# FrancisGregoryNg/Gaussian_Process_Optimization

Hardware: AMD Instinct MI355X
Metric: GP fit+predict iters/sec at N=16384 D=8 (higher is better)
Workload: dtype f64; 1 GPU; C3 (BASELINE.json configs[2]): N=16384, D=8 RBF iso, fit (K, Cholesky, alpha, LML) + predict mean/var at M=10000 candidates + EI arg-best; candidates_total=10000, candidates_this_rank=10000, entry_point=gp_fit_predict, kernel=RBF, fit=replicated on every rank (does not shard, SURVEY.md 8e), torch_imported=False, launcher=single process, emulate_fp64=0

## Files before the change

gaussian_process_optimization_amd/csrc/api_core.hip:

```cpp
#include "api_internal.h"

thread_local std::string g_err;

static thread_local bool g_note_set = false;
static thread_local std::string g_note_msg;

int fail(int code, const char *fmt, ...) {
    char buf[512];
    va_list ap;
    va_start(ap, fmt);
    vsnprintf(buf, sizeof buf, fmt, ap);
    va_end(ap);
    g_err = buf;
    if (g_note_set) {
        g_err += " [after: " + g_note_msg + "]";
        g_note_set = false;
    }
    return code;
}

void gp_note_hip(hipError_t e, const char *what, const char *file, int line) {
    if (e == hipSuccess || g_note_set) return;
    char buf[512];
    snprintf(buf, sizeof buf, "%s -> %s (%s:%d)", what, hipGetErrorString(e), file, line);
// ... 333 lines not shown
        g->panel_tiles = (int)value;
    } else if (!strcmp(name, "inner_tiles")) {
        if (value != 1 && value != 2) return fail(GP_ERR_ARG, "inner_tiles must be 1 or 2");
        g->inner_tiles = (int)value;
    } else if (!strcmp(name, "inner_min_rows")) {
        if (value < 0) return fail(GP_ERR_ARG, "inner_min_rows < 0");
        g->inner_min_rows = (int)std::min<int64_t>(value, 1 << 20);
    } else if (!strcmp(name, "own_keep_per_row")) {
        if (value < 0) return fail(GP_ERR_ARG, "own_keep_per_row < 0");
        g->own_keep_per_row = (int)std::min<int64_t>(value, 1 << 20);
    } else if (!strcmp(name, "own_keep_pipe_pct")) {
        if (value < 0 || value > 400) return fail(GP_ERR_ARG, "own_keep_pipe_pct out of range");
        g->own_keep_pipe_pct = (int)value;
    } else if (!strcmp(name, "own_keep_base")) {
        if (value < 0) return fail(GP_ERR_ARG, "own_keep_base < 0");
        g->own_keep_base = (int)std::min<int64_t>(value, 1 << 20);
    } else if (!strcmp(name, "lookahead")) {
        g->lookahead = value ? 1 : 0;
    } else if (!strcmp(name, "lookahead_min_tiles")) {
        if (value < 0) return fail(GP_ERR_ARG, "lookahead_min_tiles < 0");
        g->lookahead_min_tiles = (int)std::min<int64_t>(value, 1 << 20);
    } else if (!strcmp(name, "pipe_start_pct")) {
        if (value < -1 || value > 100) return fail(GP_ERR_ARG, "pipe_start_pct out of range");
        g->pipe_start_pct = (int)value;
    } else if (!strcmp(name, "small_below")) {
        g->small_below = (int)value;
    } else if (!strcmp(name, "profile_min_tiles")) {
        if (value < 0) return fail(GP_ERR_ARG, "profile_min_tiles < 0");
        g->profile_min_tiles = value;
    } else if (!strcmp(name, "pipe_stages_grad")) {
        if (value < 0) return fail(GP_ERR_ARG, "pipe_stages_grad < 0");
        g->pipe_stages_grad = (int)std::min<int64_t>(value, 1 << 20);
    } else if (!strcmp(name, "pipe_start_pct_grad")) {
        if (value < 0 || value > 100) return fail(GP_ERR_ARG, "pipe_start_pct_grad out of range");
        g->pipe_start_pct_grad = (int)value;
    } else if (!strcmp(name, "pipe_stages")) {
        if (value < 0) return fail(GP_ERR_ARG, "pipe_stages < 0");
        g->pipe_stages = (int)std::min<int64_t>(value, 1 << 20);
    } else if (!strcmp(name, "lauum_panels")) {
        g->lauum_panels = (int)value;
        g->wi_valid = false;
        g->li_valid = false;
        g->rows_calls_since_fit = 0;
        g->w_in_t2 = false;
    } else if (!strcmp(name, "side_alpha")) {
        g->side_alpha = (int)value;
    } else if (!strcmp(name, "pair_panels")) {
        g->pair_panels = value ? 1 : 0;
    } else if (!strcmp(name, "pair_tri")) {
        g->pair_tri = (int)value;
    } else if (!strcmp(name, "fmin_direct")) {
        g->fmin_direct = (int)value;
        g->fmin_valid = false;
    } else if (!strcmp(name, "chain_small_below")) {
        g->chain_small_below = (int)value;
    } else if (!strcmp(name, "waves8")) {
        g->waves8 = value ? 1 : 0;
    } else if (!strcmp(name, "stagger")) {
        g->stagger = (int)value;
    } else if (!strcmp(name, "supertile")) {
        if (value < 0 || value > 64) return fail(GP_ERR_ARG, "supertile out of range");
        if (g->supertile != (int)value) {
            HIPCHK(hipSetDevice(g->device));
            HIPCHK(hipDeviceSynchronize());
            for (auto &kv : g->tile_lists) hipFree(kv.second);
            g->tile_lists.clear();
        }
        g->supertile = (int)value;
    } else if (!strcmp(name, "reserve_cus")) {
        if (value != g->bulk_reserved)
            return fail(GP_ERR_ARG, "reserve_cus is fixed when the device's streams are created (%d); set GPHIP_RESERVE_CUS "
                                    "before the first gp_create", g->bulk_reserved);
    } else if (!strcmp(name, "trsm_rows64")) {
        g->trsm_rows64 = (int)value;
    } else if (!strcmp(name, "rns_interleave")) {
        rns_set_interleave((int)value);
    } else if (!strcmp(name, "rns_group_fit")) {
        if (value < 1 || value > 16) return fail(GP_ERR_ARG, "rns_group_fit must be in [1, 16]");
        g->rns_group_fit = (int)value;
    } else if (!strcmp(name, "rns_group")) {
        if (value < 1 || value > 16) return fail(GP_ERR_ARG, "rns_group must be in [1, 16]");
        g->rns_group = (int)value;
    } else if (!strcmp(name, "emulate_fit")) {
        g->emulate_fit = value ? 1 : 0;
    } else if (!strcmp(name, "emulate_fp64")) {
        g->emulate_fp64 = value ? 1 : 0;
        g->predicted = false;
    } else if (!strcmp(name, "debug_potrf_lds")) {
        if (value < 0 || value > (1 << 20)) return fail(GP_ERR_ARG, "debug_potrf_lds out of range");
        potrf_set_debug_lds((int)value);
    } else if (!strcmp(name, "debug_rows_skew")) {
        g->rows_counter_base += (unsigned int)value;
    } else if (!strcmp(name, "rows_build")) {
        if (value < -1 || value > 1) return fail(GP_ERR_ARG, "rows_build out of range (-1: by rule, 0: never, 1: at the first call)");
        g->rows_build = (int)value;
    } else if (!strcmp(name, "rows_nt")) {
        if (value < -1 || value > 1) return fail(GP_ERR_ARG, "rows_nt out of range (-1: automatic, 0, 1)");
        g->rows_nt = (int)value;
    } else if (!strcmp(name, "small_m")) {
        if (value < 0 || value > 8) return fail(GP_ERR_ARG, "small_m out of range (0..8)");
        g->small_m = value;
        g->predicted = false;
    } else if (!strcmp(name, "mc_max")) {
        if (value < GP_TILE) return fail(GP_ERR_ARG, "mc_max < 128");
        g->mc_max = round_up(value, GP_TILE);
    } else
// ... 227 lines not shown
```

gaussian_process_optimization_amd/csrc/api_factor.hip:

```cpp
#include "api_internal.h"

void build_ky(gp_ctx *g, const Members &m, bool jittered) {
    launch_kbuild(g->s, m.A, m.lda, g->dX, g->N, g->Npad, m.kp[0], m.diag[0], 0, m.nb, m.sA, m.kpt, m.diag_tab);
    if (jittered) launch_add_diag(g->s, m.A, m.lda, g->N, m.jit[0], m.nb, m.sA, m.jit_tab);
    launch_set_rhs(g->s, m.A, m.lda, g->dY, g->N, g->Npad, g->P, m.nb, m.sA);
}

static int chain_step(gp_ctx *g, hipStream_t s, const Members &m, int j, int J1, int R1) {
    double *A = m.A, *invL = m.invL;
    const long lda = m.lda;
    if (g->inner_tiles >= 2 && m.nb == 1 && j + 1 < J1 && R1 - (j + 2) >= g->inner_min_rows) {
        launch_potrf_pair(s, A, lda, j, invL, m.info);
        launch_trsm2(s, A, lda, j, invL, j + 2, R1);
        if (j + 2 < J1)
            gemm(g, s, 1, A, lda, A + (long)j * GP_TILE, lda, A + (long)j * GP_TILE, lda, 1, 2 * GP_TILE,
                 TileSet{0, R1, j + 2, J1, 1});
        return j + 2;
    }
    launch_potrf_tile(s, A, lda, j, invL, m.info, m.nb, m.sA, m.sI, 4);
    gemm(g, s, 0, A, lda, A + (long)j * GP_TILE, lda, invL + (long)j * GP_TILE * GP_TILE, GP_TILE, 0, GP_TILE,
         TileSet{j + 1, R1, j, j + 1, 0}, member_opt(m, inplace_opt(), m.sA, m.sA, m.sI));
    if (j + 1 < J1)
        gemm(g, s, 1, A, lda, A + (long)j * GP_TILE, lda, A + (long)j * GP_TILE, lda, 1, GP_TILE, TileSet{0, R1, j + 1, J1, 1},
             member_opt(m, GemmOpt(), m.sA, m.sA, m.sA));
    return j + 1;
}

void factor_buf(gp_ctx *g, const Members &m, int nt, int R1, bool side_inv) {
    const int W = g->panel_tiles;
    hipStream_t s = g->s;
    double *A = m.A;
    const long lda = m.lda;
    if (side_inv) {
        hipEvent_t e0 = la_event(g, EV_MISC, 0);
        GP_NOTE(hipEventRecord(e0, s));
        GP_NOTE(hipStreamWaitEvent(g->s_inv, e0, 0));
    }
    for (int J0 = 0; J0 < nt; J0 += W) {
        const int J1 = std::min(J0 + W, nt);
        for (int j = J0; j < J1;) j = chain_step(g, s, m, j, J1, R1);
        if (side_inv) {
            hipEvent_t eF = la_event(g, EV_CHAIN, J0 / W);
            GP_NOTE(hipEventRecord(eF, s));
            GP_NOTE(hipStreamWaitEvent(g->s_inv, eF, 0));
            build_panel_inv_one(g, g->s_inv, J0 / W, W, nt);
        }
        if (J1 < nt)
            gemm(g, s, 1, A, lda, A + (long)J0 * GP_TILE, lda, A + (long)J0 * GP_TILE, lda, 1, (J1 - J0) * GP_TILE,
                 TileSet{0, R1, J1, nt, 1}, member_opt(m, GemmOpt(), m.sA, m.sA, m.sA));
    }
    if (side_inv) {
        hipEvent_t ei = la_event(g, EV_MISC, 4);
        GP_NOTE(hipEventRecord(ei, g->s_inv));
        GP_NOTE(hipStreamWaitEvent(s, ei, 0));
    }
}

int factor(gp_ctx *g) {
    const int nt = (int)(g->Npad / GP_TILE);
    const int W = g->panel_tiles;
    const bool side = nt > W && g->s_inv;
    if (side) {
        const long PB = (long)W * GP_TILE;
        const int nJ = (nt + W - 1) / W;
        int rc;
        if ((rc = dev_realloc(&g->dInvP, &g->capInvP, (long)nJ * PB * PB))) return rc;
        if ((rc = dev_realloc(&g->dInvPw, &g->capInvPw, (long)nJ * PB * PB))) return rc;
    }
    factor_buf(g, ctx_members(g), nt, nt + 1, side);
    if (side) {
        g->invp_W = W;
        g->invp_valid = true;
        return la_events_ok(g);
    }
    return 0;
}

int factor_lookahead(gp_ctx *g, const PredPipe &pp) {
    int rc;
    if ((rc = ensure_bulk_stream(g))) return rc;
    const long lda = g->Npad;
    const int nt = (int)(g->Npad / GP_TILE);
    const int R1 = nt + 1;
    const int W = g->panel_tiles;
    double *A = g->dA;
    hipStream_t sp = g->s_panel, sb = g->s_bulk;
    hipEvent_t e0 = la_event(g, EV_MISC, 0);
    GP_NOTE(hipEventRecord(e0, g->s));
    GP_NOTE(hipStreamWaitEvent(sp, e0, 0));
    GP_NOTE(hipStreamWaitEvent(sb, e0, 0));
    const long PB = (long)W * GP_TILE;
    const int nJu = (nt + W - 1) / W;
    if ((rc = dev_realloc(&g->dInvP, &g->capInvP, (long)nJu * PB * PB))) return rc;
    if ((rc = dev_realloc(&g->dInvPw, &g->capInvPw, (long)nJu * PB * PB))) return rc;
    GP_NOTE(hipStreamWaitEvent(g->s_inv, e0, 0));
    if (pp.on) {
        GP_NOTE(hipStreamWaitEvent(g->s_pred, e0, 0));
        if (pp.init) pp.init(g->s_pred);
    }
    int next_pred = 0;
    int own_prev = nt;
    const int pstages = pp.on ? std::max(1, std::min(nJu, pp.stages)) : 0;
    const int pred_start = std::max(0, std::min(nJu - 1, nJu * pp.start_pct / 100));
    std::vector<int> pb;
    for (int j = 0; j < nt; j += W) pb.push_back(j);
    pb.push_back(nt);
    pb.push_back(nt);
    const int nJ = (int)pb.size() - 2;
    const bool emu = emu_fit_applies(g);
    RnsGeom rg;
    int *rflag = g->dInfo + 2;
    if (emu) {
        if ((rc = rns_prepare(g, g->jitter_try, &rg))) return rc;
        const long need = (long)GP_RNS_T * rg.nt256 * rg.nt256 * 65536;
        if ((rc = byte_realloc(&g->dRm, &g->capRm, need))) return rc;
    }
    const int Gf = (emu && !pp.on) ? std::max(1, std::min(g->rns_group_fit, (int)(GP_RNS_KMAX / PB))) : 1;
    hipStream_t sfar = g->s_pred;
    std::vector<char> far_issued(nJ / std::max(1, Gf) + 2, 0);
    int mid_Jg = -1, mid_end = 0, mid_first = 0, mid_base = 0, mid_next = 0;
    if (Gf > 1) GP_NOTE(hipStreamWaitEvent(sfar, e0, 0));
    const Members cm = ctx_members(g);
    for (int J = 0; J < nJ; ++J) {
        const int J0 = pb[J], J1 = pb[J + 1], J2 = pb[J + 2];
        bool bulk_recorded = false;
        for (int j = J0; j < J1;) j = chain_step(g, sp, cm, j, J1, R1);
        hipEvent_t eF = la_event(g, EV_CHAIN, J);
        GP_NOTE(hipEventRecord(eF, sp));
        const int K = (J1 - J0) * GP_TILE;
        GP_NOTE(hipStreamWaitEvent(g->s_inv, eF, 0));
        build_panel_inv_one(g, g->s_inv, J, W, nt);
        if (pp.on) {
            if (J < pstages) GP_NOTE(hipEventRecord(la_event(g, EV_INVP, J), g->s_inv));
            if (J >= pred_start) {
                for (; next_pred <= J && next_pred < pstages; ++next_pred) {
                    const int Q = next_pred, Q0 = Q * W, Q1 = std::min(Q0 + W, nt);
                    const int KQ = (Q1 - Q0) * GP_TILE;
                    const int prow = pp.trapezoid ? std::min(pp.mt, Q1) : pp.mt;
                    GP_NOTE(hipStreamWaitEvent(g->s_pred, la_event(g, EV_CHAIN, J), 0));
                    GP_NOTE(hipStreamWaitEvent(g->s_pred, la_event(g, EV_INVP, Q), 0));
                    GemmOpt o;
                    o.k_end_tri = 1;
                    o.b_sub = Q0;
                    gemm(g, g->s_pred, 0, pp.S, g->Npad, pp.T + (long)Q0 * GP_TILE, g->Npad, g->dInvP + (long)Q * PB * PB,
                         PB, 1, KQ, TileSet{0, prow, Q0, Q1, 0}, o);
                    if (Q1 < nt)
                        gemm(g, g->s_pred, 1, pp.T, g->Npad, pp.S + (long)Q0 * GP_TILE, g->Npad, A + (long)Q0 * GP_TILE, lda,
                             1, KQ, TileSet{0, prow, Q1, nt, 0});
                }
            }
        }
        if (J1 >= nt) break;
        int oc = nt;
        if (!emu && g->own_keep_per_row > 0 && J2 < nt) {
            const long n = nt - J2;
            long keep = g->own_keep_base + (long)g->own_keep_per_row * n * W / 6;
            if (pp.on && J >= pred_start && own_prev < nt) keep = keep * g->own_keep_pipe_pct / 100;
            long t_own = n * (n + 1) / 2 + n - keep;
            int c = 0;
            while (c < own_prev && (long)(c + 1) * (c + 2) / 2 + (c + 1) <= t_own) ++c;
            own_prev = c;
            oc = nt - c;
        }
        if (oc < nt && J >= 1)
            gemm(g, sp, 1, A, lda, A + (long)J0 * GP_TILE, lda, A + (long)J0 * GP_TILE, lda, 1, K, TileSet{0, R1, oc, nt, 1});
        if (J >= 1) GP_NOTE(hipStreamWaitEvent(sp, la_event(g, EV_BULK, J - 1), 0));
        gemm(g, sp, 1, A, lda, A + (long)J0 * GP_TILE, lda, A + (long)J0 * GP_TILE, lda, 1, K,
             TileSet{0, R1, J1, J2, 1});
        if (oc < nt && J == 0)
            gemm(g, sp, 1, A, lda, A + (long)J0 * GP_TILE, lda, A + (long)J0 * GP_TILE, lda, 1, K, TileSet{0, R1, oc, nt, 1});
        if (J2 < nt) {
            GP_NOTE(hipStreamWaitEvent(sb, eF, 0));
            if (emu) {
                rns_convert_panel(g, sb, rg, J, rflag);
                gemm(g, sb, 1, A, lda, A + (long)J0 * GP_TILE, lda, A + (long)J0 * GP_TILE, lda, 1, K,
                     TileSet{nt, R1, J2, nt, 0});
                auto rlaunch = [&](hipStream_t st, int Jfirst, int t0, int t1, int first, int Tend = -1) {
                    t1 = std::min(t1, nt);
                    if (t0 >= t1) return;
                    const int T0 = pb[Jfirst];
                    rns_gemm(g, st, g->dLr + (long)T0 * GP_TILE, rg.Lpitch, rg.Lplane, g->dLr + (long)T0 * GP_TILE, rg.Lpitch,
                                       rg.Lplane, g->dRm, rg.nt256, rg.nt256, rg.nt256, t0 / 2, (t1 + 1) / 2,
                                       ((Tend < 0 ? J1 : Tend) - T0) * GP_TILE, first, 1);
                };
                auto pbi = [&](int k) { return pb[std::min(k, nJ + 1)]; };
                auto rebuild_next = [&]() {
                    if (pbi(J + 2) < nt)
                        launch_rns_reconstruct256(sb, g->dRm, rg.nt256, rg.nt256, rg.nt256, pbi(J + 2), std::min(pbi(J + 3), nt),
                                                  g->Npad, A, lda, rg.back, 1);
                };
                if (Gf == 1) {
                    rlaunch(sb, J, J2, nt, J == 0 ? 1 : 0);
                    rebuild_next();
                } else {
                    const int gi = J / Gf, Jg = gi * Gf;
                    const int first = gi == 0 ? 1 : 0;
                    GP_NOTE(hipEventRecord(la_event(g, EV_CONV, J), sb));
                    rlaunch(sb, Jg, pbi(J + 2), pbi(J + 3), first);
                    rebuild_next();
                    GP_NOTE(hipEventRecord(la_event(g, EV_BULK, J), sb));
                    bulk_recorded = true;
                    if (J % Gf == Gf - 1) {
                        if (gi >= 1 && far_issued[gi - 1]) GP_NOTE(hipStreamWaitEvent(sb, la_event(g, EV_FAR, gi - 1), 0));
                        mid_Jg = Jg;
                        mid_end = J1;
                        mid_first = first;
                        mid_base = J + 3;
                        mid_next = 0;
                        if (pbi(J + 3 + Gf) < nt) {
                            GP_NOTE(hipStreamWaitEvent(sfar, la_event(g, EV_CONV, J), 0));
                            rlaunch(sfar, Jg, pbi(J + 3 + Gf), nt, first);
                            GP_NOTE(hipEventRecord(la_event(g, EV_FAR, gi), sfar));
                            far_issued[gi] = true;
                        }
                    }
                    if (mid_Jg >= 0 && mid_next < Gf) {
                        rlaunch(sb, mid_Jg, pbi(mid_base + mid_next), pbi(mid_base + mid_next + 1), mid_first, mid_end);
                        ++mid_next;
                    }
                }
            } else {
// ... 95 lines not shown

int fit_impl(gp_ctx *g, int maxtries, int pipe, int include_noise) {
    HIPCHK(hipSetDevice(g->device));
    QuiesceOnError guard{g};
    const long N = g->N, Npad = g->Npad;
    const int P = g->P;
    const int nt_ = (int)(Npad / GP_TILE);
    const long mcpad = pipe == 1 ? round_up(g->M, GP_TILE) : (pipe == 2 ? Npad : 0);
    PredPipe pp;
    if (pipe) {
        int rc;
        const int W = std::min(g->panel_tiles, nt_);
        const long PB = (long)W * GP_TILE;
        const int nJ = (nt_ + W - 1) / W;
        if (pipe == 1 && (rc = ensure_out(g))) return rc;
        if ((rc = dev_realloc(&g->dT, &g->capT, mcpad * Npad))) return rc;
        if ((rc = dev_realloc(&g->dT2, &g->capT2, mcpad * Npad))) return rc;
        if (pipe == 2 && (rc = dev_realloc(&g->dWi, &g->capWi, Npad * Npad))) return rc;
        if ((rc = dev_realloc(&g->dInvP, &g->capInvP, (long)nJ * PB * PB))) return rc;
        if ((rc = dev_realloc(&g->dInvPw, &g->capInvPw, (long)nJ * PB * PB))) return rc;
        pp.on = true;
        pp.mt = (int)(mcpad / GP_TILE);
        pp.T = g->dT;
        pp.S = g->dT2;
        pp.trapezoid = (pipe == 2);
        pp.stages = pipe == 2 ? (g->pipe_stages_grad > 0 ? g->pipe_stages_grad : std::max(1, (nJ * 36 + 50) / 100))
                              : (g->pipe_stages > 0 ? g->pipe_stages : std::max(1, (nJ * 14 + 50) / 100) + (nJ <= 12 ? 1 : 0));
        pp.start_pct = pipe == 2 ? g->pipe_start_pct_grad : (g->pipe_start_pct >= 0 ? g->pipe_start_pct : (nJ <= 24 ? 32 : 40));
    }
    double diag_add, diag0;
    ky_diag(g->kp, g->noise, &diag_add, &diag0);
    g->nphases = 0;
    g->emu_off_call = false;
    g->fitted = false;
    g->fmin_valid = false;
    g->wi_valid = false;
    g->li_valid = false;
    g->rows_calls_since_fit = 0;
    g->w_in_t2 = false;
    g->invp_valid = false;
    g->lr_valid = false;
    g->predicted = false;

    double jitter = 0.0;
    int tries = 0;
    int info = 0;
    for (;;) {
        g->lr_valid = false;
        g->jitter_try = jitter;
        int ph = phase_begin(g, "kbuild", 0.0, 8.0 * N * g->D + 8.0 * (double)N * N / 2);
        Members m = ctx_members(g);
        m.diag = &diag_add;
        m.jit = &jitter;
        build_ky(g, m, jitter != 0.0);
        phase_end(g, ph);
        HIPCHK(hipMemsetAsync(g->dInfo, 0, sizeof(int) * 4, g->s));
        if (pipe == 1) {
            pp.init = [g, mcpad, N, Npad](hipStream_t st) {
                launch_cross_k(st, g->dT, Npad, g->dXs, g->M, mcpad, g->dX, N, Npad, g->kp);
            };
            ph = phase_begin(g, "cholesky+cand_solve", (double)N * N * N / 3.0 + (double)N * N * g->M, 0.0);
            int rcf = factor_lookahead(g, pp);
            if (rcf) return rcf;
        } else if (pipe == 2) {
            ph = phase_begin(g, "cholesky+potri_stages", (double)N * N * N / 3.0, 0.0);
            pp.init = [g, Npad](hipStream_t st) { launch_set_identity(st, g->dT, Npad, Npad); };
            int rcf = factor_lookahead(g, pp);
            if (rcf) return rcf;
        } else {
            ph = phase_begin(g, "cholesky", (double)N * N * N / 3.0, 0.0);
            if (g->lookahead && nt_ > g->panel_tiles && (nt_ > g->lookahead_min_tiles || emu_fit_applies(g))) {
                int rcf = factor_lookahead(g);
                if (rcf) return rcf;
            } else {
                int rcf = factor(g);
                if (rcf) return rcf;
            }
        }
        phase_end(g, ph);
        HIPCHK(hipMemcpyAsync(&info, g->dInfo, sizeof(int), hipMemcpyDeviceToHost, g->s));
        GP_SYNC(g->s);
        if (g->emulate_fp64 && !g->emu_off_call && info == 0) {
            int bad = 0;
            HIPCHK(hipMemcpy(&bad, g->dInfo + 2, sizeof(int), hipMemcpyDeviceToHost));
            if (bad) {
                g->emu_off_call = true;
                ++g->emu_fallbacks;
                g->nphases = 0;
                g->invp_valid = false;
                continue;
            }
        }
        if (info == 0) break;
        g->invp_valid = false;
        const int rcl = ladder_step(diag0, maxtries, info, &jitter, &tries);
        if (rcl == GP_ERR_NOT_PD_DIAG) return fail(rcl, "not pd: non-positive diagonal elements");
        if (rcl) {
            g_err = "not positive definite, even with jitter.";
            return rcl;
        }
        g->nphases = 0;
    }
    g->jitter = jitter;
    bool side_alpha = false;
    if (pipe) {
        const int W = std::min(g->panel_tiles, nt_);
        const int nJ = (nt_ + W - 1) / W;
        if (g->pipe_done < nJ) {
            int phr = phase_begin(g, pipe == 2 ? "potri_solve_rest" : "cand_solve_rest", 0.0, 0.0);
            int rci = ensure_panel_inv(g);
            if (rci) return rci;
            hipEvent_t eI = la_event(g, EV_MISC, 5);
            if (g->s_inv && g->side_alpha) GP_NOTE(hipEventRecord(eI, g->s));
            solve_rows(g, ctx_members(g), (int)(mcpad / GP_TILE), pipe == 2 ? 1 : 0, g->pipe_done);
            if (g->s_inv && g->side_alpha) {
                GP_NOTE(hipStreamWaitEvent(g->s_inv, eI, 0));
                alpha_lml(g, g->s_inv, ctx_members(g));
                GP_NOTE(hipEventRecord(la_event(g, EV_MISC, 6), g->s_inv));
                side_alpha = true;
            }
            phase_end(g, phr);
        }
        if (pipe == 2) {
            int rcl = wi_lauum(g);
            if (rcl) return rcl;
// ... 73 lines not shown
```

gaussian_process_optimization_amd/csrc/api_internal.h:

```cpp
#pragma once
#include "gphip_internal.h"
#include "../../include/gphip.h"

#include <hip/hip_ext.h>
#include <rccl/rccl.h>

#include <algorithm>
#include <array>
#include <cmath>
#include <cstdarg>
#include <cstdio>
#include <cstdlib>
#include <cstring>
#include <functional>
#include <map>
#include <mutex>
#include <set>
#include <string>
#include <vector>

extern thread_local std::string g_err;
int fail(int code, const char *fmt, ...);

#define HIPCHK(x)                                                                                   \
// ... 81 lines not shown
    bool li_valid = false;
    double *dRows = nullptr;
    long capRows = 0;
    unsigned int *dRowsCounter = nullptr;
    double *hRowsOut = nullptr;
    double rows_ticket = 0.0;
    unsigned int rows_counter_base = 0;
    std::vector<double> lp_cache;
    int lp_cache_nb = -1;
    long rows_fused_calls = 0, rows_fallback_calls = 0;
    long rows_calls_since_fit = 0;
    int rows_build = -1;
    int rows_nt = -1;
    double *dLp = nullptr;
    double *dX2 = nullptr, *dK2 = nullptr;
    long capX2 = 0, capK2 = 0;
    long capLp = 0;
    double *dCov = nullptr;
    long capCov = 0;
    double *dInvP = nullptr, *dInvPw = nullptr;
    long capInvP = 0, capInvPw = 0;
    int invp_W = 0;
    bool invp_valid = false;
    double *dDm = nullptr, *dDv = nullptr, *dDacq = nullptr;
    long capD = 0;
    int panel_tiles = 6;
    int lookahead = 1;
    int inner_min_rows = 0;
    int own_keep_per_row = 36, own_keep_base = 200;
    int own_keep_pipe_pct = 0;
    int inner_tiles = 1;
    int lookahead_min_tiles = 40;
    int reserve_cus = 32;
    long mc_max = 16384;
    long small_m = 8;
    Phase phases[MAX_PHASES];
    int nphases = 0;
    bool profiling = false;
    int profile_class = 0;
    std::vector<hipEvent_t> gemm_events;
    std::vector<hipEvent_t> rns_events;
    size_t rns_ev_used = 0;
    double rns_ops = 0.0;
    std::vector<long> gemm_tiles;
    std::map<std::array<int, 5>, short *> tile_lists;
    int supertile = 8;
    int small_below = 1400;
    int chain_small_below = 400;
    int lauum_panels = 1;
    int side_alpha = 1;
    int pair_panels = 1;
    int pair_tri = 2;
    int fmin_direct = 0;
    int trsm_rows64 = 32;
    int waves8 = 1;
    int stagger = 3;
    int pipe_stages_grad = 0, pipe_start_pct_grad = 40;
    int pipe_stages = 0;
    int pipe_done = 0;
    int pipe_start_pct = -1;
    std::vector<int> gemm_K;
    size_t gemm_ev_used = 0;
    long gemm_launches = 0;
    double gemm_flops = 0.0;
    double gemm_flops_all = 0.0;
    long profile_min_tiles = 1024;
    ncclComm_t comm = nullptr;
    int rank = 0, nranks = 1;
    double *dComm = nullptr;
    long capComm = 0;
    int emulate_fp64 = 0;
    int rns_group = 8;
    int rns_group_fit = 8;
    signed char *dLr = nullptr, *dSr = nullptr, *dRr = nullptr;
    signed char *dRm = nullptr;
    signed char *dWr = nullptr;
    long capWr = 0;
    long capLr = 0, capSr = 0, capRr = 0, capRm = 0;
    bool lr_valid = false;
    std::vector<char> lr_done;
    int lr_W = 0, lr_e = 0;
    double jitter_try = 0.0;
    int emulate_fit = 1;
    bool emu_off_call = false;
    long emu_fallbacks = 0;
    double *dBatch = nullptr;
    long capBatch = 0;
    signed char *dBatchAux = nullptr;
    long capBatchAux = 0;
    bool dead = false;
};

static inline long round_up(long x, long m) { return (x + m - 1) / m * m; }

static inline bool emu_fit_applies(const gp_ctx *g) {
    const long PB = (long)g->panel_tiles * GP_TILE;
    return g->emulate_fp64 && g->emulate_fit && !g->emu_off_call && (PB % 256 == 0) && PB <= GP_RNS_KMAX;
}

static inline GemmOpt inplace_opt() {
    GemmOpt o;
    o.inplace = 1;
    return o;
}

struct Members {
// ... 12 lines not shown
    const double *diag = nullptr, *diag_tab = nullptr;
    const double *jit = nullptr, *jit_tab = nullptr;
};
Members ctx_members(gp_ctx *g);
Members members_range(const Members &m, int m0, int nb);
static inline GemmOpt member_opt(const Members &m, GemmOpt o, long sC, long sA, long sB) {
    o.batch = o.members = m.nb;
    o.sC = sC;
    o.sA = sA;
    o.sB = sB;
    return o;
}

struct PredPipe {
    bool on = false;
    int mt = 0;
    double *T = nullptr, *S = nullptr;
    std::function<void(hipStream_t)> init;
    bool trapezoid = false;
    int stages = 0, start_pct = 0;
};

struct RnsGeom {
    int e = 0;
    double scale = 1.0, back = 1.0;
    long Lrows = 0, Lplane = 0, Lpitch = 0;
    int nt256 = 0;
};

struct RnsSolveOpt {
    bool trapezoid = false;
    int eS = -1;
    signed char *Wr = nullptr;
    long wpitch = 0, wplane = 0;
};

struct DevStreams {
    hipStream_t s = nullptr, panel = nullptr, bulk = nullptr, inv = nullptr, pred = nullptr;
    int reserved = -1;
};

enum { EV_CHAIN = 0, EV_BULK = 1, EV_INVP = 2, EV_MISC = 3, EV_FAR = 4, EV_CONV = 5 };

void shutdown_all();
int make_bulk_stream(int device, int reserve, hipStream_t *out);
int get_streams(int device, int reserve, DevStreams *out);
int phase_begin(gp_ctx *g, const char *name, double flops, double bytes);
void phase_end(gp_ctx *g, int id);
void gemm(gp_ctx *g, hipStream_t s, int mode, double *C, long ldc, const double *A, long lda, const double *B, long ldb, int b_mul, int K, TileSet ts, const GemmOpt &o = GemmOpt());
void rns_gemm(gp_ctx *g, hipStream_t s, const signed char *A, long lda, long a_plane, const signed char *B, long ldb, long b_plane, signed char *R, int mt_all, int nt_all, int mt, int c0, int c1, int K, int first, int tri = 0);
int dev_realloc(double **p, long *cap, long need);
void destroy_ctx_events(gp_ctx *g);
void build_ky(gp_ctx *g, const Members &m, bool jittered);
void factor_buf(gp_ctx *g, const Members &m, int nt, int R1, bool side_inv = false);
int factor(gp_ctx *g);
void alpha_lml(gp_ctx *g, hipStream_t s, const Members &m);
void ky_diag(const KernParams &kp, double noise, double *diag_add, double *diag0);
int ladder_step(double diag0, int maxtries, int info, double *jitter, int *tries);
double lml_from_scalars(long N, int P, const double *scal);
void build_panel_inv_one(gp_ctx *g, hipStream_t s, int J, int W, int nt);
int byte_realloc(signed char **p, long *cap, long need);
int rns_prepare(gp_ctx *g, double jitter, RnsGeom *r);
void rns_convert_panel(gp_ctx *g, hipStream_t s, const RnsGeom &r, int J, int *flag);
int factor_lookahead(gp_ctx *g, const PredPipe &pp = PredPipe());
int ensure_bulk_stream(gp_ctx *g);
hipEvent_t la_event(gp_ctx *g, int kind, size_t i);
int la_events_ok(gp_ctx *g);
int ensure_panel_inv(gp_ctx *g);
void identity_blocks(hipStream_t s, double *T, long n, int nb);
void panel_inv_members(gp_ctx *g, const Members &m);
void solve_rows(gp_ctx *g, const Members &m, int mt, int trapezoid, int J_from = 0);
int solve_rows_rns(gp_ctx *g, double *T, double *S, int mt, const RnsSolveOpt &opt = RnsSolveOpt());
int fit_impl(gp_ctx *g, int maxtries, int pipe, int include_noise);
int run_predict(gp_ctx *g, int include_noise, bool tiles_only = false);
int ensure_out(gp_ctx *g);
int run_acq(gp_ctx *g, int type, double par, double fmin, double y_mean, double y_std);
struct LpBatch { double *X = nullptr, *r = nullptr, *s = nullptr; };
int upload_lp_batch(gp_ctx *g, const double *Xb, int nb, const double *r0, const double *s0, LpBatch *b);
int run_acq_lp(gp_ctx *g, int type, double par, double fmin, double y_mean, double y_std, int transform, const double *Xb, int nb, const double *r0, const double *s0);
void lauum(gp_ctx *g, const Members &m);
int wi_lauum(gp_ctx *g);
int wi_rns(gp_ctx *g);
int ensure_wi(gp_ctx *g);
int ensure_linv(gp_ctx *g);
void lml_grad_passes(gp_ctx *g, const Members &m);
void grads_from_sums(const double *h, const KernParams &kp, int ard, double *dvariance, double *dlengthscale, double *dnoise);
int lml_grad_impl(gp_ctx *g, double *dvariance, double *dlengthscale, double *dnoise, bool reset_phases);
int ensure_grad_buffers(gp_ctx *g, long elemsBeta, long M);
int run_predict_grad(gp_ctx *g);
```

gaussian_process_optimization_amd/csrc/gphip_internal.h:

```cpp
#pragma once
#include <hip/hip_runtime.h>
#include <stdint.h>
#include <algorithm>
#include <string>
#include <vector>

#define GP_TILE 128
#define GP_MAX_RHS 128

typedef double double4_t __attribute__((ext_vector_type(4)));
typedef double double2_t __attribute__((ext_vector_type(2)));

void gp_note_hip(hipError_t e, const char *what, const char *file, int line);
#define GP_NOTE(call) gp_note_hip((call), #call, __FILE__, __LINE__)
#define GP_LAUNCH(kernel, grid, block, lds, stream, ...)                                   \
    do {                                                                                   \
        (void)hipGetLastError();  \
        hipLaunchKernelGGL(kernel, grid, block, lds, stream, __VA_ARGS__);                 \
        gp_note_hip(hipGetLastError(), #kernel, __FILE__, __LINE__);                       \
    } while (0)

#define GP_MAX_D 64
struct KernParams {
    int kernel;
// ... 35 lines not shown
__device__ __forceinline__ void gp_k_and_g(int kernel, double variance, double r2, double &k, double &g) {
    if (kernel == 0) {
        k = variance * gp_exp_nonpos(-0.5 * r2);
        g = -k;
    } else {
        const double s5 = 2.23606797749978969640917366873128;
        const double r = sqrt(r2);
        const double e = gp_exp_nonpos(-s5 * r);
        k = variance * (1.0 + s5 * r + (5.0 / 3.0) * r2) * e;
        g = -(5.0 / 3.0) * variance * (1.0 + s5 * r) * e;
    }
}

__host__ __device__ static inline double kp_div(const KernParams &kp, int d) { return kp.gower ? kp.gdiv[d] : kp.ls[d]; }

struct TileSet {
    int r0, r1, c0, c1, tri;
};
static inline long tileset_count(const TileSet &t) {
    if (!t.tri) return (long)(t.r1 - t.r0) * (t.c1 - t.c0);
    long n = 0;
    for (int c = t.c0; c < t.c1; ++c) n += (t.r1 - c) > 0 ? (t.r1 - c) : 0;
    return n;
}

struct GemmOpt {
    int k_tri = 0;
    int k_sub = 0;
    int k_end_tri = 0;
    int b_sub = 0;
    int batch = 1;
    int members = 1;
    long sC = 0, sA = 0, sB = 0;
    const short *tile_list = nullptr;
    int stagger = 0;
    int small = 0;
    int waves8 = 0;
    int inplace = 0;
    int rows64 = 0;
    int pair = 0;
};
std::vector<short> build_tile_list(const TileSet &ts, int S);
void launch_gemm_nt(hipStream_t s, int mode, double *C, long ldc, const double *A, long lda,
                    const double *B, long ldb, int b_mul, int K, TileSet ts, const GemmOpt &o = GemmOpt());

void launch_potrf_tile(hipStream_t s, double *A, long lda, int t, double *invL, int *info, int nb = 1, long sA = 0, long sI = 0,
                       int sInfo = 0);
void launch_potrf_pair(hipStream_t s, double *A, long lda, int t, double *invL, int *info);
void launch_trsm2(hipStream_t s, double *A, long lda, int t, const double *invL, int r0, int r1);
void potrf_set_debug_lds(int bytes);


void launch_kbuild(hipStream_t s, double *A, long lda, const double *X, long N, long Npad, const KernParams &kp, double diag_add,
                   int full, int nb = 1, long sA = 0, const KernParams *kpt = nullptr, const double *diag_tab = nullptr);
void launch_set_rhs(hipStream_t s, double *A, long lda, const double *Y, long N, long Npad, int P, int nb = 1, long sA = 0);
void launch_cross_k(hipStream_t s, double *T, long ldt, const double *Xs, long M, long Mpad,
                    const double *X, long N, long Npad, const KernParams &kp);

void launch_cross_k_rows(hipStream_t s, double *T, long ldt, const double *Xs, int M, const double *X, long N, long Npad,
                         const KernParams &kp);

void launch_logdet(hipStream_t s, const double *A, long lda, long N, double *out, int nb = 1, long sA = 0, long so = 0);
void launch_rhs_sumsq(hipStream_t s, const double *A, long lda, long N, long Npad, int P, double *out);

void launch_trsv_backward(hipStream_t s, const double *L, long lda, const double *invP, int W, long Npad, const double *Z, long ldz,
                          int P, double *Aout, double *w, int nb = 1, long sL = 0, long sP = 0, long sV = 0);

void launch_predict_reduce(hipStream_t s, const double *T, long ldt, long M, long N, const double *Z,
                           long ldz, int P, double kss, double noise_add, double *mean, double *var);

void launch_train_mean(hipStream_t s, const double *X, long N, const KernParams &kp, const double *alpha,
                       double *mu);
void launch_train_mean_identity(hipStream_t s, const double *Y, const double *alpha, double d, long N, double *mu);
void launch_min(hipStream_t s, const double *v, long n, double *out);

void launch_acq(hipStream_t s, int type, double par, double fmin, double y_mean, double y_std,
                const double *mean, const double *var, long M, double *out);
void launch_argbest(hipStream_t s, const double *v, long n, int sense, double *best_val, long long *best_idx,
                    double *scratch_val, long long *scratch_idx);

void launch_small_forward_solve(hipStream_t s, const double *L, long lda, const double *invP, int W, long Npad, double *T,
                                double *S, long ldt, int M);
void launch_small_wi_product(hipStream_t s, const double *Wi, long ldw, long Npad, const double *Kx, long ldk, int M,
                             double *beta, long ldb);

#define ROWS_MAX_M 4
#define ROWS_MAX_XS 128
struct RowsX {
    int M;
    double xs[ROWS_MAX_XS];
};
struct RowsAcq {
    int on;
    int type;
    double par, fmin, y_mean, y_std;
    int lp, transform, nb;
    const double *Xb, *r0, *s0;
};
#define ROWS_OUT_DOUBLES (3 * ROWS_MAX_M * (1 + GP_MAX_D))
struct RowsWork {
    double *wpart, *bpart, *meanpart, *vpart, *gpart;
    unsigned int *counter;
    unsigned int counter_base;
    double ticket;
};
long rows_tiles(int nt);
int rows_block_height(int nt);
// ... 50 lines not shown
```

gaussian_process_optimization_amd/csrc/kbuild.hip:

```cpp
#include "gphip_internal.h"

#define k_of_r2 gp_k_of_r2
__device__ __forceinline__ double gower_factor(int kernel, double variance, double dx, int disc) {
    const double r = disc ? (dx != 0.0 ? 1.0 : 0.0) : fabs(dx);
    return k_of_r2(kernel, variance, r * r);
}

__device__ __forceinline__ void stage_rows_T(double *dst, const double *X, long row0, long N, int D,
                                             const double *ls, int tid) {
    for (int idx = tid; idx < GP_TILE * D; idx += 256) {
        const int r = idx / D, d = idx - r * D;
        const long g = row0 + r;
        dst[d * GP_TILE + r] = (g < N) ? X[g * D + d] / ls[d] : 0.0;
    }
}

template <int DU>
__device__ __forceinline__ void kbuild_body(double *A, long lda, const double *X, long N, long Npad, const KernParams &kp,
                                            double diag_add, int full, int nt) {
    extern __shared__ __attribute__((aligned(16))) double sm[];
    const int DS = DU > 0 ? DU : kp.D;
    double *xi = sm;
    double *xj = sm + (long)DS * GP_TILE;
    __shared__ double ils[GP_MAX_D];
    const int tid = threadIdx.x;
    int tm, tn;
    if (full) {
        tm = blockIdx.x / nt;
        tn = blockIdx.x % nt;
    } else {
        const long t = blockIdx.x;
        tm = (int)((sqrt(8.0 * (double)t + 1.0) - 1.0) * 0.5);
        while ((long)tm * (tm + 1) / 2 > t) --tm;
        while ((long)(tm + 1) * (tm + 2) / 2 <= t) ++tm;
        tn = (int)(t - (long)tm * (tm + 1) / 2);
    }
    if (tid < kp.D) ils[tid] = kp_div(kp, tid);
    __syncthreads();
    stage_rows_T(xi, X, (long)tm * GP_TILE, N, kp.D, ils, tid);
    stage_rows_T(xj, X, (long)tn * GP_TILE, N, kp.D, ils, tid);
    if (DU > 0)
        for (int idx = kp.D * GP_TILE + tid; idx < DU * GP_TILE; idx += 256) xi[idx] = xj[idx] = 0.0;
    __syncthreads();

    const int cx = (tid & 63) * 2;
    const int ry = tid >> 6;
    const long gc = (long)tn * GP_TILE + cx;
    double2_t bq[DU > 0 ? DU : 1];
    if (DU > 0) {
#pragma unroll
        for (int d = 0; d < DU; ++d) bq[d] = *(const double2_t *)(xj + d * GP_TILE + cx);
    }
    for (int q = 0; q < 32; ++q) {
        const int r = ry + 4 * q;
        const long gr = (long)tm * GP_TILE + r;
        double2_t out;
        if (kp.gower) {
            double p0 = 1.0, p1 = 1.0;
            for (int d = 0; d < kp.D; ++d) {
                const double a = xi[d * GP_TILE + r];
                const double2_t b = *(const double2_t *)(xj + d * GP_TILE + cx);
                p0 *= gower_factor(kp.kernel, kp.variance, a - b[0], kp.gdisc[d]);
                p1 *= gower_factor(kp.kernel, kp.variance, a - b[1], kp.gdisc[d]);
            }
            out[0] = p0;
            out[1] = p1;
        } else {
            double s0 = 0.0, s1 = 0.0;
            if (DU > 0) {
#pragma unroll
                for (int d = 0; d < DU; ++d) {
                    const double a = xi[d * GP_TILE + r];
                    const double d0 = a - bq[d][0], d1 = a - bq[d][1];
                    s0 = fma(d0, d0, s0);
                    s1 = fma(d1, d1, s1);
                }
            } else {
                for (int d = 0; d < kp.D; ++d) {
                    const double a = xi[d * GP_TILE + r];
                    const double2_t b = *(const double2_t *)(xj + d * GP_TILE + cx);
                    const double d0 = a - b[0], d1 = a - b[1];
                    s0 = fma(d0, d0, s0);
                    s1 = fma(d1, d1, s1);
                }
            }
            out[0] = k_of_r2(kp.kernel, kp.variance, s0);
            out[1] = k_of_r2(kp.kernel, kp.variance, s1);
        }
        if (gr >= N) {
            out[0] = (gr == gc) ? 1.0 : 0.0;
            out[1] = (gr == gc + 1) ? 1.0 : 0.0;
        } else {
            if (gc >= N) out[0] = 0.0;
            else if (gr == gc) out[0] = (kp.gower ? out[0] : kp.variance) + diag_add;
            if (gc + 1 >= N) out[1] = 0.0;
            else if (gr == gc + 1) out[1] = (kp.gower ? out[1] : kp.variance) + diag_add;
        }
        *(double2_t *)(A + gr * lda + gc) = out;
    }
}

template <int DU>
__global__ __launch_bounds__(256) void kbuild_kernel(double *A, long lda, const double *X, long N, long Npad,
                                                     KernParams kp, double diag_add, int full, int nt) {
    kbuild_body<DU>(A, lda, X, N, Npad, kp, diag_add, full, nt);
}
template <int DU>
__global__ __launch_bounds__(256) void kbuild_batch_kernel(double *A, long lda, long sA, const double *X, long N, long Npad,
                                                           const KernParams *kpt, const double *diag_add, int nt) {
    const long z = blockIdx.z;
    kbuild_body<DU>(A + z * sA, lda, X, N, Npad, kpt[z], diag_add[z], 0, nt);
}

static void launch_kbuild_members(hipStream_t s, double *A, long lda, long sA, const double *X, long N, long Npad, int DU, size_t shm,
                                  const KernParams *kpt, const double *diag_tab, int nb);

void launch_kbuild(hipStream_t s, double *A, long lda, const double *X, long N, long Npad, const KernParams &kp, double diag_add,
                   int full, int nb, long sA, const KernParams *kpt, const double *diag_tab) {
    const int nt = (int)(Npad / GP_TILE);
    const long nblk = full ? (long)nt * nt : (long)nt * (nt + 1) / 2;
    const int DU = kp.gower ? 0 : (kp.D <= 8 ? 8 : (kp.D <= 16 ? 16 : 0));
    const size_t shm = (size_t)2 * (DU ? DU : kp.D) * GP_TILE * sizeof(double);
    if (nb > 1) return launch_kbuild_members(s, A, lda, sA, X, N, Npad, DU, shm, kpt, diag_tab, nb);
    if (DU == 8)
        GP_LAUNCH(kbuild_kernel<8>, dim3((unsigned)nblk), dim3(256), shm, s, A, lda, X, N, Npad, kp, diag_add, full, nt);
    else if (DU == 16)
        GP_LAUNCH(kbuild_kernel<16>, dim3((unsigned)nblk), dim3(256), shm, s, A, lda, X, N, Npad, kp, diag_add, full, nt);
    else
        GP_LAUNCH(kbuild_kernel<0>, dim3((unsigned)nblk), dim3(256), shm, s, A, lda, X, N, Npad, kp, diag_add, full, nt);
}

__device__ __forceinline__ void set_rhs_body(double *A, long lda, const double *Y, long N, long Npad, int P) {
    const long i = (long)blockIdx.x * blockDim.x + threadIdx.x;
    const int p = blockIdx.y;
    if (i >= Npad) return;
    A[(Npad + p) * lda + i] = (p < P && i < N) ? Y[i * P + p] : 0.0;
}
__global__ void set_rhs_kernel(double *A, long lda, const double *Y, long N, long Npad, int P) {
    set_rhs_body(A, lda, Y, N, Npad, P);
}
__global__ void set_rhs_batch_kernel(double *A, long lda, long sA, const double *Y, long N, long Npad, int P) {
    set_rhs_body(A + (long)blockIdx.z * sA, lda, Y, N, Npad, P);
}

void launch_set_rhs(hipStream_t s, double *A, long lda, const double *Y, long N, long Npad, int P, int nb, long sA) {
    if (nb > 1) {
        dim3 grid((unsigned)((Npad + 255) / 256), GP_MAX_RHS, (unsigned)nb);
        GP_LAUNCH(set_rhs_batch_kernel, grid, dim3(256), 0, s, A, lda, sA, Y, N, Npad, P);
        return;
    }
    dim3 grid((unsigned)((Npad + 255) / 256), GP_MAX_RHS);
    GP_LAUNCH(set_rhs_kernel, grid, dim3(256), 0, s, A, lda, Y, N, Npad, P);
}

template <int DU>
__global__ __launch_bounds__(256) void cross_k_kernel(double *T, long ldt, const double *Xs, long M, const double *X,
                                                      long N, KernParams kp, int nti) {
    extern __shared__ __attribute__((aligned(16))) double sm[];
    const int DS = DU > 0 ? DU : kp.D;
    double *xc = sm;
    double *xt = sm + (long)DS * GP_TILE;
    __shared__ double ils[GP_MAX_D];
    const int tid = threadIdx.x;
    const int tc = blockIdx.x / nti, ti = blockIdx.x % nti;
    if (tid < kp.D) ils[tid] = kp_div(kp, tid);
    __syncthreads();
    stage_rows_T(xc, Xs, (long)tc * GP_TILE, M, kp.D, ils, tid);
    stage_rows_T(xt, X, (long)ti * GP_TILE, N, kp.D, ils, tid);
    if (DU > 0)
        for (int idx = kp.D * GP_TILE + tid; idx < DU * GP_TILE; idx += 256) xc[idx] = xt[idx] = 0.0;
    __syncthreads();
    const int cx = (tid & 63) * 2;
    const int ry = tid >> 6;
    const long gi = (long)ti * GP_TILE + cx;
    double2_t bq[DU > 0 ? DU : 1];
    if (DU > 0) {
#pragma unroll
        for (int d = 0; d < DU; ++d) bq[d] = *(const double2_t *)(xt + d * GP_TILE + cx);
    }
    for (int q = 0; q < 32; ++q) {
        const int r = ry + 4 * q;
        const long gcand = (long)tc * GP_TILE + r;
// ... 102 lines not shown
```

Baseline: 14.73 fit+predict iters/s.

## Split kernel-matrix build so factorization starts after the first panel columns

After: 14.82 fit+predict iters/s, median of 6. Within noise of the previous version (+0.6%).

```diff
diff --git a/gaussian_process_optimization_amd/csrc/api_core.hip b/gaussian_process_optimization_amd/csrc/api_core.hip
--- a/gaussian_process_optimization_amd/csrc/api_core.hip
+++ b/gaussian_process_optimization_amd/csrc/api_core.hip
@@ -409,6 +409,9 @@
     } else if (!strcmp(name, "fmin_direct")) {
         g->fmin_direct = (int)value;
         g->fmin_valid = false;
+    } else if (!strcmp(name, "kbuild_split")) {
+        if (value < 0 || value > 2) return fail(GP_ERR_ARG, "kbuild_split out of range (0: one launch, 1, 2: two)");
+        g->kbuild_split = (int)value;
     } else if (!strcmp(name, "chain_small_below")) {
         g->chain_small_below = (int)value;
     } else if (!strcmp(name, "waves8")) {
diff --git a/gaussian_process_optimization_amd/csrc/api_factor.hip b/gaussian_process_optimization_amd/csrc/api_factor.hip
--- a/gaussian_process_optimization_amd/csrc/api_factor.hip
+++ b/gaussian_process_optimization_amd/csrc/api_factor.hip
@@ -4,6 +4,12 @@
     launch_kbuild(g->s, m.A, m.lda, g->dX, g->N, g->Npad, m.kp[0], m.diag[0], 0, m.nb, m.sA, m.kpt, m.diag_tab);
     if (jittered) launch_add_diag(g->s, m.A, m.lda, g->N, m.jit[0], m.nb, m.sA, m.jit_tab);
     launch_set_rhs(g->s, m.A, m.lda, g->dY, g->N, g->Npad, g->P, m.nb, m.sA);
+}
+
+void build_ky_head(gp_ctx *g, const Members &m, const KyTail &t) {
+    launch_kbuild(g->s, m.A, m.lda, g->dX, g->N, g->Npad, m.kp[0], t.diag_add, 0, 1, 0, nullptr, nullptr, t.head_tiles);
+    launch_set_rhs(g->s, m.A, m.lda, g->dY, g->N, g->Npad, g->P, 1, 0);
+    GP_NOTE(hipEventRecord(t.e_head, g->s));
 }
 
 static int chain_step(gp_ctx *g, hipStream_t s, const Members &m, int j, int J1, int R1) {
@@ -76,7 +82,7 @@
     return 0;
 }
 
-int factor_lookahead(gp_ctx *g, const PredPipe &pp) {
+int factor_lookahead(gp_ctx *g, const PredPipe &pp, const KyTail *tail) {
     int rc;
     if ((rc = ensure_bulk_stream(g))) return rc;
     const long lda = g->Npad;
@@ -86,8 +92,16 @@
     double *A = g->dA;
     hipStream_t sp = g->s_panel, sb = g->s_bulk;
     hipEvent_t e0 = la_event(g, EV_MISC, 0);
-    GP_NOTE(hipEventRecord(e0, g->s));
-    GP_NOTE(hipStreamWaitEvent(sp, e0, 0));
+    if (tail) {
+        hipStream_t st = tail->on_bulk ? sb : g->s;
+        GP_NOTE(hipStreamWaitEvent(sp, tail->e_head, 0));
+        if (tail->on_bulk) GP_NOTE(hipStreamWaitEvent(sb, tail->e_head, 0));
+        launch_kbuild(st, A, lda, g->dX, g->N, g->Npad, g->kp, tail->diag_add, 0, 1, 0, nullptr, nullptr, -tail->head_tiles);
+        GP_NOTE(hipEventRecord(e0, st));
+    } else {
+        GP_NOTE(hipEventRecord(e0, g->s));
+        GP_NOTE(hipStreamWaitEvent(sp, e0, 0));
+    }
     GP_NOTE(hipStreamWaitEvent(sb, e0, 0));
     const long PB = (long)W * GP_TILE;
     const int nJu = (nt + W - 1) / W;
@@ -167,6 +181,7 @@
         if (J >= 1) GP_NOTE(hipStreamWaitEvent(sp, la_event(g, EV_BULK, J - 1), 0));
         gemm(g, sp, 1, A, lda, A + (long)J0 * GP_TILE, lda, A + (long)J0 * GP_TILE, lda, 1, K,
              TileSet{0, R1, J1, J2, 1});
+        if (tail && J == 0) GP_NOTE(hipStreamWaitEvent(sp, e0, 0));
         if (oc < nt && J == 0)
             gemm(g, sp, 1, A, lda, A + (long)J0 * GP_TILE, lda, A + (long)J0 * GP_TILE, lda, 1, K, TileSet{0, R1, oc, nt, 1});
         if (J2 < nt) {
@@ -368,25 +383,35 @@
         Members m = ctx_members(g);
         m.diag = &diag_add;
         m.jit = &jitter;
-        build_ky(g, m, jitter != 0.0);
+        const bool la_route = pipe || (g->lookahead && nt_ > g->panel_tiles && (nt_ > g->lookahead_min_tiles || emu_fit_applies(g)));
+        KyTail tail;
+        if (la_route && g->kbuild_split && jitter == 0.0 && !emu_fit_applies(g) && 2 * g->panel_tiles < nt_) {
+            tail.head_tiles = 2 * g->panel_tiles;
+            tail.e_head = la_event(g, EV_MISC, 8);
+            tail.diag_add = diag_add;
+            tail.on_bulk = g->kbuild_split >= 2;
+        }
+        const KyTail *tailp = tail.head_tiles ? &tail : nullptr;
+        HIPCHK(hipMemsetAsync(g->dInfo, 0, sizeof(int) * 4, g->s));
+        if (tailp) build_ky_head(g, m, tail);
+        else build_ky(g, m, jitter != 0.0);
         phase_end(g, ph);
-        HIPCHK(hipMemsetAsync(g->dInfo, 0, sizeof(int) * 4, g->s));
         if (pipe == 1) {
             pp.init = [g, mcpad, N, Npad](hipStream_t st) {
                 launch_cross_k(st, g->dT, Npad, g->dXs, g->M, mcpad, g->dX, N, Npad, g->kp);
             };
             ph = phase_begin(g, "cholesky+cand_solve", (double)N * N * N / 3.0 + (double)N * N * g->M, 0.0);
-            int rcf = factor_lookahead(g, pp);
+            int rcf = factor_lookahead(g, pp, tailp);
             if (rcf) return rcf;
         } else if (pipe == 2) {
             ph = phase_begin(g, "cholesky+potri_stages", (double)N * N * N / 3.0, 0.0);
             pp.init = [g, Npad](hipStream_t st) { launch_set_identity(st, g->dT, Npad, Npad); };
-            int rcf = factor_lookahead(g, pp);
+            int rcf = factor_lookahead(g, pp, tailp);
             if (rcf) return rcf;
         } else {
             ph = phase_begin(g, "cholesky", (double)N * N * N / 3.0, 0.0);
-            if (g->lookahead && nt_ > g->panel_tiles && (nt_ > g->lookahead_min_tiles || emu_fit_applies(g))) {
-                int rcf = factor_lookahead(g);
+            if (la_route) {
+                int rcf = factor_lookahead(g, PredPipe(), tailp);
                 if (rcf) return rcf;
             } else {
                 int rcf = factor(g);
diff --git a/gaussian_process_optimization_amd/csrc/api_internal.h b/gaussian_process_optimization_amd/csrc/api_internal.h
--- a/gaussian_process_optimization_amd/csrc/api_internal.h
+++ b/gaussian_process_optimization_amd/csrc/api_internal.h
@@ -157,6 +157,7 @@
     int pair_panels = 1;
     int pair_tri = 2;
     int fmin_direct = 0;
+    int kbuild_split = 2;
     int trsm_rows64 = 32;
     int waves8 = 1;
     int stagger = 3;
@@ -275,6 +276,13 @@
 int dev_realloc(double **p, long *cap, long need);
 void destroy_ctx_events(gp_ctx *g);
 void build_ky(gp_ctx *g, const Members &m, bool jittered);
+struct KyTail {
+    int head_tiles = 0;
+    hipEvent_t e_head = nullptr;
+    double diag_add = 0.0;
+    bool on_bulk = false;
+};
+void build_ky_head(gp_ctx *g, const Members &m, const KyTail &t);
 void factor_buf(gp_ctx *g, const Members &m, int nt, int R1, bool side_inv = false);
 int factor(gp_ctx *g);
 void alpha_lml(gp_ctx *g, hipStream_t s, const Members &m);
@@ -285,7 +293,8 @@
 int byte_realloc(signed char **p, long *cap, long need);
 int rns_prepare(gp_ctx *g, double jitter, RnsGeom *r);
 void rns_convert_panel(gp_ctx *g, hipStream_t s, const RnsGeom &r, int J, int *flag);
-int factor_lookahead(gp_ctx *g, const PredPipe &pp = PredPipe());
+struct KyTail;
+int factor_lookahead(gp_ctx *g, const PredPipe &pp = PredPipe(), const KyTail *tail = nullptr);
 int ensure_bulk_stream(gp_ctx *g);
 hipEvent_t la_event(gp_ctx *g, int kind, size_t i);
 int la_events_ok(gp_ctx *g);
diff --git a/gaussian_process_optimization_amd/csrc/gphip_internal.h b/gaussian_process_optimization_amd/csrc/gphip_internal.h
--- a/gaussian_process_optimization_amd/csrc/gphip_internal.h
+++ b/gaussian_process_optimization_amd/csrc/gphip_internal.h
@@ -111,7 +111,7 @@
 
 
 void launch_kbuild(hipStream_t s, double *A, long lda, const double *X, long N, long Npad, const KernParams &kp, double diag_add,
-                   int full, int nb = 1, long sA = 0, const KernParams *kpt = nullptr, const double *diag_tab = nullptr);
+                   int full, int nb = 1, long sA = 0, const KernParams *kpt = nullptr, const double *diag_tab = nullptr, int csplit = 0);
 void launch_set_rhs(hipStream_t s, double *A, long lda, const double *Y, long N, long Npad, int P, int nb = 1, long sA = 0);
 void launch_cross_k(hipStream_t s, double *T, long ldt, const double *Xs, long M, long Mpad,
                     const double *X, long N, long Npad, const KernParams &kp);
diff --git a/gaussian_process_optimization_amd/csrc/kbuild.hip b/gaussian_process_optimization_amd/csrc/kbuild.hip
--- a/gaussian_process_optimization_amd/csrc/kbuild.hip
+++ b/gaussian_process_optimization_amd/csrc/kbuild.hip
@@ -17,7 +17,7 @@
 
 template <int DU>
 __device__ __forceinline__ void kbuild_body(double *A, long lda, const double *X, long N, long Npad, const KernParams &kp,
-                                            double diag_add, int full, int nt) {
+                                            double diag_add, int full, int nt, int csplit = 0) {
     extern __shared__ __attribute__((aligned(16))) double sm[];
     const int DS = DU > 0 ? DU : kp.D;
     double *xi = sm;
@@ -30,10 +30,20 @@
         tn = blockIdx.x % nt;
     } else {
         const long t = blockIdx.x;
-        tm = (int)((sqrt(8.0 * (double)t + 1.0) - 1.0) * 0.5);
-        while ((long)tm * (tm + 1) / 2 > t) --tm;
-        while ((long)(tm + 1) * (tm + 2) / 2 <= t) ++tm;
-        tn = (int)(t - (long)tm * (tm + 1) / 2);
+        const long tri = csplit > 0 ? (long)csplit * (csplit + 1) / 2 : 0;
+        if (csplit > 0 && t >= tri) {
+            tm = csplit + (int)((t - tri) / csplit);
+            tn = (int)((t - tri) % csplit);
+        } else {
+            tm = (int)((sqrt(8.0 * (double)t + 1.0) - 1.0) * 0.5);
+            while ((long)tm * (tm + 1) / 2 > t) --tm;
+            while ((long)(tm + 1) * (tm + 2) / 2 <= t) ++tm;
+            tn = (int)(t - (long)tm * (tm + 1) / 2);
+            if (csplit < 0) {
+                tm -= csplit;
+                tn -= csplit;
+            }
+        }
     }
     if (tid < kp.D) ils[tid] = kp_div(kp, tid);
     __syncthreads();
@@ -102,8 +112,8 @@
 
 template <int DU>
 __global__ __launch_bounds__(256) void kbuild_kernel(double *A, long lda, const double *X, long N, long Npad,
-                                                     KernParams kp, double diag_add, int full, int nt) {
-    kbuild_body<DU>(A, lda, X, N, Npad, kp, diag_add, full, nt);
+                                                     KernParams kp, double diag_add, int full, int nt, int csplit) {
+    kbuild_body<DU>(A, lda, X, N, Npad, kp, diag_add, full, nt, csplit);
 }
 template <int DU>
 __global__ __launch_bounds__(256) void kbuild_batch_kernel(double *A, long lda, long sA, const double *X, long N, long Npad,
@@ -116,18 +126,21 @@
                                   const KernParams *kpt, const double *diag_tab, int nb);
 
 void launch_kbuild(hipStream_t s, double *A, long lda, const double *X, long N, long Npad, const KernParams &kp, double diag_add,
-                   int full, int nb, long sA, const KernParams *kpt, const double *diag_tab) {
+                   int full, int nb, long sA, const KernParams *kpt, const double *diag_tab, int csplit) {
     const int nt = (int)(Npad / GP_TILE);
-    const long nblk = full ? (long)nt * nt : (long)nt * (nt + 1) / 2;
+    if (full || nb > 1 || csplit >= nt || -csplit >= nt) csplit = 0;
+    const long c = csplit > 0 ? csplit : -csplit, rest = nt - c;
+    const long nblk = full ? (long)nt * nt
+                           : (csplit > 0 ? c * (c + 1) / 2 + rest * c : (csplit < 0 ? rest * (rest + 1) / 2 : (long)nt * (nt + 1) / 2));
     const int DU = kp.gower ? 0 : (kp.D <= 8 ? 8 : (kp.D <= 16 ? 16 : 0));
     const size_t shm = (size_t)2 * (DU ? DU : kp.D) * GP_TILE * sizeof(double);
     if (nb > 1) return launch_kbuild_members(s, A, lda, sA, X, N, Npad, DU, shm, kpt, diag_tab, nb);
     if (DU == 8)
-        GP_LAUNCH(kbuild_kernel<8>, dim3((unsigned)nblk), dim3(256), shm, s, A, lda, X, N, Npad, kp, diag_add, full, nt);
+        GP_LAUNCH(kbuild_kernel<8>, dim3((unsigned)nblk), dim3(256), shm, s, A, lda, X, N, Npad, kp, diag_add, full, nt, csplit);
     else if (DU == 16)
-        GP_LAUNCH(kbuild_kernel<16>, dim3((unsigned)nblk), dim3(256), shm, s, A, lda, X, N, Npad, kp, diag_add, full, nt);
+        GP_LAUNCH(kbuild_kernel<16>, dim3((unsigned)nblk), dim3(256), shm, s, A, lda, X, N, Npad, kp, diag_add, full, nt, csplit);
     else
-        GP_LAUNCH(kbuild_kernel<0>, dim3((unsigned)nblk), dim3(256), shm, s, A, lda, X, N, Npad, kp, diag_add, full, nt);
+        GP_LAUNCH(kbuild_kernel<0>, dim3((unsigned)nblk), dim3(256), shm, s, A, lda, X, N, Npad, kp, diag_add, full, nt, csplit);
 }
 
 __device__ __forceinline__ void set_rhs_body(double *A, long lda, const double *Y, long N, long Npad, int P) {
```
